# swoonge/SC-A-LOAM

Measured on AMD Instinct MI355X. Metric: scans/sec (feat-extract + scan-to-map ICP + SC loop search), KITTI HDL-64, higher is better.
Workload: dtype f32 points / f64 pose algebra

## Files before the change

sc-a-loam_amd/csrc/mapping.hip:

```cpp
#include "common.hpp"
#include <mutex>
#include <atomic>
#include "device_utils.hpp"
#include "voxel_dev.hpp"
#include "radix_sort.hpp"
#include "lm_host.hpp"
#include "features_dev.hpp"
#include <cmath>
#include <cstdlib>
#include <algorithm>
#include <deque>

namespace scal {

constexpr int CW = 21, CH = 21, CD = 11;
constexpr int GX = 250, GY = 250, GZ = 150;
constexpr int GCELLS = GX * GY * GZ;
constexpr unsigned long long MAP_NOMERGE = 127ull;

struct MapParams {
    int cenW, cenH, cenD;
    int cI, cJ, cK;
    int ox, oy, oz;
    float inv_line, inv_plane;
// ... 663 lines not shown
        C->n_total[cls] = min(n_old + ns, cap);
        if (n_old + ns > cap) C->error = SCAL_E_CAPACITY;
    }
    if (i >= n_old + ns || i >= cap) return;
    float x, y, z;
    int pc;
    if (i < n_old) {
        x = m.x[i], y = m.y[i], z = m.z[i], pc = m.cube[i];
    } else {
        const int j = i - n_old;
        double x7[7];
#pragma unroll
        for (int k = 0; k < 7; ++k) x7[k] = st->x[k];
        float sel[3];
        associate_to_map(x7, stack.x[j], stack.y[j], stack.z[j], sel);
        x = sel[0], y = sel[1], z = sel[2];
        pc = pack_cube(cube_abs(x) , cube_abs(y), cube_abs(z));
        m.x[i] = x, m.y[i] = y, m.z[i] = z, m.w[i] = stack.w[j], m.cube[i] = pc;
    }
    const unsigned long long k = map_key(mp, inv_leaf, x, y, z, pc, C);
    keys[i] = k;
    vals[i] = i;
}
SCAL_KERNEL(256, k_insert_keys)

__device__ __forceinline__ void k_map_heads_body(const SortedPairs& sp, const int* __restrict__ d_n, int* __restrict__ blockcnt) {
    const unsigned long long* keys = sp.keys[sorted_sel(sp)];
    const int n = *d_n;
    const int nb = (n + 255) / 256;
    if (static_cast<int>(blockIdx.x) >= nb) return;
    __shared__ int s[17];
    const int i = blockIdx.x * 256 + threadIdx.x;
    int head = 0;
    if (i < n) {
        const unsigned long long k = keys[i];
        head = (k != ~0ull) && (((k >> 27) == MAP_NOMERGE) || i == 0 || keys[i - 1] != k);
    }
    int total;
    block_exclusive_scan(head, s, &total);
    if (threadIdx.x == 0) blockcnt[blockIdx.x] = total;
}
SCAL_KERNEL(256, k_map_heads)

__device__ __forceinline__ void k_map_reduce_body(const SortedPairs& sp, const int* __restrict__ d_n, const int* __restrict__ blockoff, const MapCloud& in,
                                                    const MapCloud& out) {
    const unsigned long long* keys = sp.keys[sorted_sel(sp)];
    const int* vals = sp.vals[sorted_sel(sp)];
    const int n = *d_n;
    const int nb = (n + 255) / 256;
    if (static_cast<int>(blockIdx.x) >= nb) return;
    __shared__ int s[17];
    const int i = blockIdx.x * 256 + threadIdx.x;
    int head = 0;
    unsigned long long k = 0;
    if (i < n) {
        k = keys[i];
        head = (k != ~0ull) && (((k >> 27) == MAP_NOMERGE) || i == 0 || keys[i - 1] != k);
    }
    int total;
    const int rank = block_exclusive_scan(head, s, &total);
    if (!head) return;
    const int o = blockoff[blockIdx.x] + rank;
    if ((k >> 27) == MAP_NOMERGE) {
        const int g = vals[i];
        out.x[o] = in.x[g], out.y[o] = in.y[g], out.z[o] = in.z[g], out.w[o] = in.w[g], out.cube[o] = in.cube[g];
        return;
    }
    float ax = 0.f, ay = 0.f, az = 0.f, aw = 0.f;
    int u = i;
    while (u < n && keys[u] == k) {
        const int g = vals[u];
        ax += in.x[g], ay += in.y[g], az += in.z[g], aw += in.w[g];
        ++u;
    }
    const float c = static_cast<float>(u - i);
    out.x[o] = ax / c, out.y[o] = ay / c, out.z[o] = az / c, out.w[o] = aw / c;
    out.cube[o] = in.cube[vals[i]];
}
SCAL_KERNEL(256, k_map_reduce)

constexpr int MERGE_MAX = 16384;
constexpr int MERGE_IDX_BITS = 14;
constexpr int MERGE_SAMPLES = 4096;

struct MergeNew {
    float *x, *y, *z, *w;
    int* cube;
    unsigned long long* pkey;
    unsigned long long* sorted;
    unsigned long long* samp;
    int* pre;
    int* lb;
    unsigned char* hm;
    int* blocktot;
};
struct MergeArgs {
    MapCloud in[2], out[2];
    CSoA4 stack[2];
    const int* d_ns[2];
    float inv_leaf[2];
    unsigned long long* okeys[2];
    MergeNew nw[2];
    int cap;
    int2* grid_cell[2];
    const int* grid_rank[2];
    int prebuild;
    int2* next_cell[2];
    int* next_rank[2];
    float4* next_pool[2];
    unsigned long long* next_okeys[2];
    int next_cap[2];
};
constexpr int MERGE_CHUNKS = MERGE_MAX / 512;
constexpr int MERGE_KB0 = 24, MERGE_KB1 = 88;
constexpr int MERGE_KEYS_GRID = 2 * MERGE_CHUNKS;
constexpr int MERGE_NEW_BLOCKS = MERGE_MAX / 256;
constexpr int MERGE_WB0 = 256, MERGE_WB1 = 1536;
constexpr int MERGE_WRITE_GRID = MERGE_WB0 + MERGE_WB1 + 2 * MERGE_NEW_BLOCKS;


__device__ __forceinline__ void k_merge_okeys_body(const MergeArgs& a, const MapState* __restrict__ S, MapCounters* C) {
    if (S->abort) return;
    const MapParams mp = S->mp;
    int b = blockIdx.x;
    const int cls = b < MERGE_KB0 ? 0 : 1;
    const int nblk = cls ? MERGE_KB1 : MERGE_KB0;
    if (cls) b -= MERGE_KB0;
    const MapCloud m = a.in[cls];
    const int n_old = S->n_map[cls];
    for (int i = b * 1024 + threadIdx.x; i < n_old; i += nblk * 1024) {
        const unsigned long long k = map_key(mp, a.inv_leaf[cls], m.x[i], m.y[i], m.z[i], m.cube[i], C);
        a.okeys[cls][i] = k;
        bool bad = k == ~0ull;
        if (i > 0) {
            const unsigned long long kp = map_key(mp, a.inv_leaf[cls], m.x[i - 1], m.y[i - 1], m.z[i - 1], m.cube[i - 1], C);
            bad |= kp > k || (kp == k && !key_nomerge(k));
        }
        if (bad) C->merge_fail = 1;
    }
}
SCAL_KERNEL(1024, k_merge_okeys)

__device__ __forceinline__ void k_merge_keys_body(const MergeArgs& a, const LMState* __restrict__ st, MapState* S, MapCounters* C) {
    if (S->abort) return;
    if (blockIdx.x == 0 && threadIdx.x == 0) S->next_valid[0] = 0, S->next_valid[1] = 0, S->next_unsorted = 0, S->next_over = 0;
    extern __shared__ __align__(16) unsigned long long sk[];
    __shared__ int s_scan[17];
    int b = blockIdx.x;
    const int cls = b / MERGE_CHUNKS, tile = b % MERGE_CHUNKS;
    const int ns = *a.d_ns[cls];
    const int n_new = min(ns, MERGE_MAX);
    const int nc = (n_new + 511) >> 9;
    if (tile == 0 && threadIdx.x == 0 && (ns > MERGE_MAX || S->n_map[cls] + ns > a.cap || !S->window_same)) C->merge_fail = 1;
    if (tile > 0 && tile >= nc) return;
    const MergeNew nw = a.nw[cls];
    int mine = 0;
    for (int i = threadIdx.x; i < nc * 512; i += 1024) {
        const unsigned long long pk = i < n_new ? nw.pkey[i] : ~0ull;
        mine += pk != ~0ull;
        sk[i] = pk;
    }
    int n_eff = 0;
    block_exclusive_scan(mine, s_scan, &n_eff);
    if (tile == 0 && threadIdx.x == 0) C->merge_neff[cls] = n_eff;
    if (nc == 0) return;
    for (int w = wave_id(); w < nc; w += 16) {
        unsigned long long v[8];
        chunk_load(sk, w, v);
        wave_sort512(v);
        chunk_store(sk, w, v);
    }
    __syncthreads();
    const int j = threadIdx.x >> 1, half = threadIdx.x & 1;
    const unsigned long long key = sk[tile * 512 + j];
    int rank = half == 0 ? j : 0;
    for (int c = half; c < nc; c += 2) {
        if (c == tile) continue;
        const unsigned long long* ch = sk + c * 512;
        int lo = 0, hi = 512;
        while (lo < hi) {
            const int mid = (lo + hi) >> 1;
            if (ch[mid] < key) lo = mid + 1;
            else hi = mid;
        }
        rank += lo;
    }
    rank += __shfl_xor(rank, 1, 64);
    if (half == 0 && key != ~0ull) nw.sorted[rank] = key;
}
SCAL_KERNEL(1024, k_merge_keys)

__device__ __forceinline__ void k_merge_lookup_body(const MergeArgs& a, const MapState* __restrict__ S, const MapCounters* __restrict__ C) {
    if (S->abort) return;
    __shared__ unsigned long long s_samp[MERGE_SAMPLES];
    __shared__ int s_scan[17];
    const int cls = blockIdx.x / MERGE_CHUNKS, blk = blockIdx.x % MERGE_CHUNKS;
    const MergeNew nw = a.nw[cls];
    const int n_eff = C->merge_neff[cls];
    if (blk * 512 >= n_eff) {
        if (threadIdx.x == 0) nw.blocktot[blk] = 0;
        return;
    }
    const int n_old = S->n_map[cls];
    const unsigned long long* okeys = a.okeys[cls];
    int stride = 32;
    while ((n_old + stride - 1) / stride > MERGE_SAMPLES) stride <<= 1;
    const int n_samp = (n_old + stride - 1) / stride;
    for (int j = threadIdx.x; j < n_samp; j += 512) s_samp[j] = okeys[static_cast<size_t>(j) * stride];
    const int t = blk * 512 + threadIdx.x;
    unsigned long long key = 0;
    bool head = false, nom = false;
    int lo = 0, hi = 0;
    if (t < n_eff) {
        key = nw.sorted[t] >> MERGE_IDX_BITS;
        nom = key_nomerge(key);
        head = nom || t == 0 || (nw.sorted[t - 1] >> MERGE_IDX_BITS) != key;
        if (head && !nom) hi = n_old;
        if (nom) lo = hi = n_old;
    }
    __syncthreads();
    if (lo < hi) {
        int x = 0, y = n_samp;
        while (x < y) {
            const int mid = (x + y) >> 1;
            if (s_samp[mid] < key) x = mid + 1;
            else y = mid;
        }
        lo = x > 0 ? (x - 1) * stride + 1 : 0;
        hi = min(n_old, x * stride);
        if (lo > hi) lo = hi;
        while (lo < hi) {
            const int mid = (lo + hi) >> 1;
            if (okeys[mid] < key) lo = mid + 1;
            else hi = mid;
        }
    }
    const bool matched = head && !nom && lo < n_old && okeys[lo] == key;
    const int ins = (head && !matched) ? 1 : 0;
    int total = 0;
    const int pre = block_exclusive_scan(ins, s_scan, &total);
    if (t < n_eff) {
        nw.hm[t] = (head ? 1 : 0) | (matched ? 2 : 0);
        nw.lb[t] = lo;
        nw.pre[t] = pre;
        if ((t & 7) == 0) nw.samp[t >> 3] = key;
    }
    if (threadIdx.x == 0) nw.blocktot[blk] = total;
}
SCAL_KERNEL(512, k_merge_lookup)

__device__ __forceinline__ void merge_write_body(const MergeArgs& a, MapState* S, MapCounters* C) {
    if (S->abort) return;
    if (static_cast<int>(blockIdx.x) < MERGE_WB0 + MERGE_WB1) {
        const int cls0 = static_cast<int>(blockIdx.x) < MERGE_WB0 ? 0 : 1;
        const int b0 = cls0 ? blockIdx.x - MERGE_WB0 : blockIdx.x, nblk0 = cls0 ? MERGE_WB1 : MERGE_WB0;
        const MapParams mp0 = S->mp;
        const MapCloud m0 = a.in[cls0];
        const int n0 = S->n_map[cls0];
        for (int i = b0 * 256 + threadIdx.x; i < n0; i += nblk0 * 256)
            if (a.grid_rank[cls0][i] >= 0) a.grid_cell[cls0][grid_cell(mp0, m0.x[i], m0.y[i], m0.z[i])].x = 0;
    }
    if (C->merge_fail) {
        if (blockIdx.x == 0 && threadIdx.x == 0) __hip_atomic_store(&S->abort, static_cast<int>(MAP_ABORT_MERGE), __ATOMIC_RELAXED, __HIP_MEMORY_SCOPE_AGENT);
        return;
    }
    if (static_cast<int>(blockIdx.x) >= MERGE_WRITE_GRID) return;
    __shared__ int s_base[MERGE_CHUNKS + 1];
    __shared__ unsigned long long s_samp[MERGE_MAX / 8];
    int b = blockIdx.x;
    int cls, part, nblk;
    if (b < MERGE_WB0) cls = 0, part = 0, nblk = MERGE_WB0;
    else if ((b -= MERGE_WB0) < MERGE_WB1) cls = 1, part = 0, nblk = MERGE_WB1;
    else if ((b -= MERGE_WB1) < MERGE_NEW_BLOCKS) cls = 0, part = 1, nblk = MERGE_NEW_BLOCKS;
    else b -= MERGE_NEW_BLOCKS, cls = 1, part = 1, nblk = MERGE_NEW_BLOCKS;
    const MapCloud in = a.in[cls], out = a.out[cls];
    const MergeNew nw = a.nw[cls];
    const int n_eff = C->merge_neff[cls];
    const int n_old = S->n_map[cls];
    if (part == 0 && b * 256 >= n_old && b > 0) return;
    const int n_samp = (n_eff + 7) >> 3;
    if (part == 0)
        for (int q = threadIdx.x; q < n_samp; q += 256) s_samp[q] = nw.samp[q];
    if (threadIdx.x < MERGE_CHUNKS) s_base[threadIdx.x + 1] = nw.blocktot[threadIdx.x];
    __shared__ int s_valid;
    if (threadIdx.x == 0) s_valid = 0;
    __syncthreads();
    if (threadIdx.x == 0) {
        int run = 0;
        for (int q = 0; q < MERGE_CHUNKS; ++q) {
            const int v = s_base[q + 1];
            s_base[q] = run;
            run += v;
        }
        s_base[MERGE_CHUNKS] = run;
    }
    __syncthreads();
    const int total = s_base[MERGE_CHUNKS];
    if (n_old + total > a.cap) {
        if (b == 0 && part == 0 && threadIdx.x == 0) __hip_atomic_store(&S->abort, static_cast<int>(MAP_ABORT_MERGE), __ATOMIC_RELAXED, __HIP_MEMORY_SCOPE_AGENT);
        return;
    }
    if (b == 0 && part == 0 && threadIdx.x == 0) __hip_atomic_store(&C->n_map_new[cls], n_old + total, __ATOMIC_RELAXED, __HIP_MEMORY_SCOPE_AGENT);
    auto pre_at = [&](int t) { return t < n_eff ? nw.pre[t] + s_base[t >> 9] : total; };
    const MapParams mp = S->mp;
    bool drifted = false, over = false;
    int n_in = 0;
    auto prebuild = [&](int o, float x, float y, float z, int cube, unsigned long long placed) {
        const unsigned long long k = map_key(mp, a.inv_leaf[cls], x, y, z, cube, C);
        a.next_okeys[cls][o] = k;
        drifted |= k != placed;
        if (cube_valid(mp, cube)) {
            ++n_in;
            const int cap = a.next_cap[cls];
            const int c = grid_cell(mp, x, y, z);
            const int r = atomicAdd(&a.next_cell[cls][c].x, 1);
            a.next_rank[cls][o] = r;
            if (r < cap) {
                a.next_pool[cls][static_cast<size_t>(c) * cap + r] = make_float4(x, y, z, __int_as_float(o));
                if (r == 0) a.next_cell[cls][c].y = c * cap;
            } else {
                over = true;
            }
        } else {
            a.next_rank[cls][o] = -1;
        }
    };
    if (part == 0) {
        for (int i = b * 256 + threadIdx.x; i < n_old; i += nblk * 256) {
            const unsigned long long k = a.okeys[cls][i];
            const float ix = in.x[i], iy = in.y[i], iz = in.z[i], iw = in.w[i];
            const int cube = in.cube[i];
            int lo, hi;
            {
                int x = 0, y = n_samp;
                while (x < y) {
                    const int mid = (x + y) >> 1;
                    if (s_samp[mid] < k) x = mid + 1;
                    else y = mid;
                }
                lo = x > 0 ? (x - 1) * 8 + 1 : 0;
                hi = min(n_eff, x * 8);
                if (lo > hi) lo = hi;
            }
            unsigned long long e[8];
#pragma unroll
            for (int j = 0; j < 8; ++j) e[j] = lo + j < n_eff ? nw.sorted[lo + j] : ~0ull;
            int cn = 0;
#pragma unroll
            for (int j = 0; j < 7; ++j) cn += (lo + j < hi && (e[j] >> MERGE_IDX_BITS) < k) ? 1 : 0;
            const int at = lo + cn;
            const int o = i + pre_at(at);
            float ax = 0.f, ay = 0.f, az = 0.f, aw = 0.f;
            ax += ix, ay += iy, az += iz, aw += iw;
            int cnt = 1;
            if (!key_nomerge(k)) {
                bool run = true;
#pragma unroll
                for (int j = 0; j < 8; ++j)
                    if (j >= cn) {
                        run = run && (e[j] >> MERGE_IDX_BITS) == k;
                        if (run) {
                            const int jn = static_cast<int>(e[j] & (MERGE_MAX - 1));
                            ax += nw.x[jn], ay += nw.y[jn], az += nw.z[jn], aw += nw.w[jn];
                            ++cnt;
                        }
                    }
                if (run) {
                    int u = lo + 8;
                    while (u < n_eff && (nw.sorted[u] >> MERGE_IDX_BITS) == k) {
                        const int jn = static_cast<int>(nw.sorted[u] & (MERGE_MAX - 1));
                        ax += nw.x[jn], ay += nw.y[jn], az += nw.z[jn], aw += nw.w[jn];
                        ++u, ++cnt;
                    }
                }
            }
            const float c = static_cast<float>(cnt);
            const float ox = ax / c, oy = ay / c, oz = az / c;
            out.x[o] = ox, out.y[o] = oy, out.z[o] = oz, out.w[o] = aw / c, out.cube[o] = cube;
            if (a.prebuild) prebuild(o, ox, oy, oz, cube, k);
        }
    } else {
        const int i = b * 256 + threadIdx.x;
        if (i < n_eff && (nw.hm[i] & 3) == 1) {
            const unsigned long long k = nw.sorted[i] >> MERGE_IDX_BITS;
            const int o = nw.lb[i] + pre_at(i);
            float ax = 0.f, ay = 0.f, az = 0.f, aw = 0.f;
// ... 40 lines not shown
    merge_write_body(a, S, C);
    if (!t.fused) return;
    if (static_cast<int>(blockIdx.x) >= MERGE_WRITE_GRID && S->pose_seq == t.seq) {
        const int i = (blockIdx.x - MERGE_WRITE_GRID) * 256 + threadIdx.x;
        if (i < min(*t.d_nfull, t.full_cap)) {
            double x7[7];
#pragma unroll
            for (int k = 0; k < 7; ++k) x7[k] = t.st->x[k];
            float sel[3];
            associate_to_map(x7, t.full.x[i], t.full.y[i], t.full.z[i], sel);
            t.full_out.x[i] = sel[0], t.full_out.y[i] = sel[1], t.full_out.z[i] = sel[2], t.full_out.w[i] = t.full.w[i];
        }
    }
}
SCAL_KERNEL(256, k_merge_write)

__device__ __forceinline__ void k_transform_cloud_body(const CSoA4& in, const int* __restrict__ d_n, int cap, const LMState* __restrict__ st,
                                                         const MapState* __restrict__ S, const SoA4& out) {
    if (S->abort) return;
    const int i = blockIdx.x * blockDim.x + threadIdx.x;
    if (i >= min(*d_n, cap)) return;
    double x7[7];
#pragma unroll
    for (int k = 0; k < 7; ++k) x7[k] = st->x[k];
    float sel[3];
    associate_to_map(x7, in.x[i], in.y[i], in.z[i], sel);
    out.x[i] = sel[0], out.y[i] = sel[1], out.z[i] = sel[2], out.w[i] = in.w[i];
}
SCAL_KERNEL(256, k_transform_cloud)

__device__ __forceinline__ void k_map_gather_body(const float* __restrict__ less_aos, const int* __restrict__ d_n_less, const CSoA4& less_flat,
                                                    const int* __restrict__ d_n_less_flat, const SoA4& corner_in, const SoA4& surf_in, MapCounters* C, int cap,
                                                    int nbc, unsigned* surf_parts) {
    const bool corner = static_cast<int>(blockIdx.x) < nbc;
    const int b = corner ? blockIdx.x : blockIdx.x - nbc;
    const int n = min(corner ? *d_n_less : *d_n_less_flat, cap);
    const int i = b * 256 + threadIdx.x;
    if (blockIdx.x == 0) {
        int* w = reinterpret_cast<int*>(C);
        for (int t = 2 + threadIdx.x; t < static_cast<int>(sizeof(MapCounters) / sizeof(int)); t += 256) w[t] = 0;
    }
    if (i == 0) (corner ? C->n_corner_in : C->n_surf_in) = n;
    if (corner) {
        if (i >= n) return;
        const float4 p = reinterpret_cast<const float4*>(less_aos)[i];
        corner_in.x[i] = p.x, corner_in.y[i] = p.y, corner_in.z[i] = p.z, corner_in.w[i] = p.w;
    } else {
        float x = 0.f, y = 0.f, z = 0.f;
        if (i < n) {
            x = less_flat.x[i], y = less_flat.y[i], z = less_flat.z[i];
            surf_in.x[i] = x, surf_in.y[i] = y, surf_in.z[i] = z, surf_in.w[i] = less_flat.w[i];
        }
        if (surf_parts) vox_bbox_block_store(surf_parts, b, i < n, x, y, z);
    }
}
SCAL_KERNEL(256, k_map_gather)

__device__ __forceinline__ void k_export_valid_body(const MapCloud& m, const MapState* __restrict__ S, int cls, int* __restrict__ counter,
                                                      float* __restrict__ out, int cap) {
    const MapParams mp = S->mp;
    const int n = S->n_map[cls];
    for (int i = blockIdx.x * blockDim.x + threadIdx.x; i < n; i += gridDim.x * blockDim.x)
        if (cube_valid(mp, m.cube[i])) {
            const int p = atomicAdd(counter, 1);
            if (p < cap) reinterpret_cast<float4*>(out)[p] = make_float4(m.x[i], m.y[i], m.z[i], m.w[i]);
        }
}
SCAL_KERNEL(256, k_export_valid)


__device__ __forceinline__ void copy_words(void* dst, const void* src, int bytes) {
    const unsigned* s = static_cast<const unsigned*>(src);
    unsigned* d = static_cast<unsigned*>(dst);
    for (int i = threadIdx.x; i < bytes / 4; i += blockDim.x) d[i] = s[i];
}

struct PoseDoneNew {
    CSoA4 stack[2];
    const int* d_ns[2];
    float inv_leaf[2];
    float *x[2], *y[2], *z[2], *w[2];
    int* cube[2];
    unsigned long long* pkey[2];
};
struct MapPoseDone {
    int active;
    unsigned seq;
    MapState* S;
    const LMState* st;
    MapCounters* C;
    MapResult* host;
    PoseDoneNew nw;
    __device__ __forceinline__ void operator()(const double* x, int first, int stride, bool aborted) const {
        if (!active) return;
        const bool stop = aborted || S->abort;
        if (!stop) {
            const MapParams mp = S->mp;
            double x7[7];
#pragma unroll
            for (int k = 0; k < 7; ++k) x7[k] = x[k];
#pragma unroll
            for (int cls = 0; cls < 2; ++cls) {
                const int n_new = min(*nw.d_ns[cls], MERGE_MAX);
                const CSoA4 stack = nw.stack[cls];
                for (int i = first; i < n_new; i += stride) {
                    float sel[3];
                    associate_to_map(x7, stack.x[i], stack.y[i], stack.z[i], sel);
                    const int pc = pack_cube(cube_abs(sel[0]), cube_abs(sel[1]), cube_abs(sel[2]));
                    const unsigned long long k = map_key(mp, nw.inv_leaf[cls], sel[0], sel[1], sel[2], pc, C);
                    nw.x[cls][i] = sel[0], nw.y[cls][i] = sel[1], nw.z[cls][i] = sel[2], nw.w[cls][i] = stack.w[i], nw.cube[cls][i] = pc;
                    nw.pkey[cls][i] = k == ~0ull ? ~0ull : ((k << MERGE_IDX_BITS) | static_cast<unsigned long long>(i));
                }
            }
        }
        if (blockIdx.x != 0) return;
        if (first == 0 && !stop) {
            const double* q_wodom = S->q_wodom;
            const double n2 = q_wodom[0] * q_wodom[0] + q_wodom[1] * q_wodom[1] + q_wodom[2] * q_wodom[2] + q_wodom[3] * q_wodom[3];
            const double qi[4] = {-q_wodom[0] / n2, -q_wodom[1] / n2, -q_wodom[2] / n2, q_wodom[3] / n2};
            double qn[4];
            q_mul(x, qi, qn);
            double r2[3];
            q_rot(qn, S->t_wodom, r2);
#pragma unroll
            for (int i = 0; i < 4; ++i) S->q_wmap_wodom[i] = qn[i];
#pragma unroll
            for (int i = 0; i < 3; ++i) S->t_wmap_wodom[i] = x[4 + i] - r2[i];
            S->pose_seq = seq;
        }
        __syncthreads();
        copy_words(&host->st, st, sizeof(LMState));
        copy_words(&host->C1, C, sizeof(MapCounters));
        copy_words(&host->S1, S, sizeof(MapState));
        __threadfence_system();
        __syncthreads();
        if (threadIdx.x == 0) __hip_atomic_store(&host->seq_pose, seq, __ATOMIC_RELEASE, __HIP_MEMORY_SCOPE_SYSTEM);
    }
    __device__ __forceinline__ void operator()(int, int, int) const {}
};

__device__ __forceinline__ void k_map_pose_done_body(const MapPoseDone& pd) {
    pd(pd.st->x, blockIdx.x * blockDim.x + threadIdx.x, gridDim.x * blockDim.x, false);
}
SCAL_KERNEL(256, k_map_pose_done)

__device__ __forceinline__ void k_map_end_body(MapState* S, const MapCounters* C, MapResult* host, unsigned seq) {
    if (threadIdx.x == 0 && !S->abort) S->n_map[0] = C->n_map_new[0], S->n_map[1] = C->n_map_new[1];
    __syncthreads();
    copy_words(&host->C2, C, sizeof(MapCounters));
    copy_words(&host->S2, S, sizeof(MapState));
    __threadfence_system();
    __syncthreads();
    if (threadIdx.x == 0) __hip_atomic_store(&host->seq_done, seq, __ATOMIC_RELEASE, __HIP_MEMORY_SCOPE_SYSTEM);
}
SCAL_KERNEL(256, k_map_end)

struct MapStore {
    SoAStore pts[2];
    DevBuf<int> cube[2];
    int n = 0;
    MapCloud cloud(int b) { return MapCloud{pts[b].x.p, pts[b].y.p, pts[b].z.p, pts[b].w.p, cube[b].p}; }
};

struct GridStore {
    DevBuf<int2> cell[2];
    DevBuf<int> rank[2];
    DevBuf<float4> g;
    DevBuf<float4> fixed[2];
    DevBuf<unsigned long long> okeys[2];
    int fixed_cap = 0;
    GridPts pts(int par, bool fixed_pool = false) { return GridPts{fixed_pool ? fixed[par].p : g.p}; }
};

SCAL_DEFINE_STAMP_READER(scal_debug_stamps_map)
}

using namespace scal;
// ... 19 lines not shown
    bool pose_collected = false;
    bool confirmed = false;
    bool failed = false;
    bool prebuilt = false;
    unsigned seq = 0;
    unsigned feat_generation = 0;
    int n_corner_bound = 0, n_surf_bound = 0;
    int insert_path = 0;
};

struct InputSet {
    SoAStore in[2], stack[2];
    DevBuf<MapCounters> C;
    DevBuf<unsigned> surf_parts;
    Event ev_pre;
    Event ev_pre_a;
    int* n_in(int k) const { return k == 0 ? &C.p->n_corner_in : &C.p->n_surf_in; }
    int* n_stack(int k) const { return k == 0 ? &C.p->n_corner_stack : &C.p->n_surf_stack; }
};

template <class T, int N>
struct Fifo {
    T item[N];
    int n = 0;
    void push(const T& v) { item[n++] = v; }
    const T& front() const { return item[0]; }
    void pop() { std::copy(item + 1, item + n, item), --n; }
    void clear() { n = 0; }
};

struct scal_map {
    scal_map_config cfg;
    LaneStream stream;
    LaneStream side;
    static constexpr int NSETS = 8;
    static constexpr int MAX_STEPS = 4;
    static constexpr int MAX_PF = 3;
    static constexpr int NSLOTS = MAX_STEPS + 1;
    struct Prefetch {
        scal_features_t* feat;
        int set;
        unsigned generation;
    };
    std::mutex pf_mu;
    Fifo<Prefetch, MAX_PF> pf_half;
    Fifo<Prefetch, MAX_PF> pf;
    int next_set = 0;
    std::deque<MapStep> steps;
    Event ev_pose[NSLOTS], ev_done[NSLOTS];
    int next_slot = 0;
    PinBuf<MapResult> res;
    bool adapter_active = false;
    MapStep adapter_step;
    BlockAdapter blocks;
    int n_fast = 0, n_general = 0, n_recover_pose = 0, n_recover_insert = 0;
    bool poll_on_enqueue = true;
    int cur = 0;
    bool initialised = false;
    double good_q[4] = {0, 0, 0, 1}, good_t[3] = {0, 0, 0};
    int scan_cap = 0, map_cap = 0;
    double q_wmap_wodom[4] = {0, 0, 0, 1}, t_wmap_wodom[3] = {0, 0, 0};
    bool have_mp = false;
    DevBuf<MapState> d_S;
    DevBuf<float> aos;
    DevBuf<float> export_buf;
    InputSet sets[NSETS];
    SoAStore full_in, full_out;
    float leaf(int k) const { return k == 0 ? cfg.line_res : cfg.plane_res; }
    float inv_leaf(int k) const { return 1.0f / leaf(k); }
    VoxelFilter vf, vf_side, vf_corner;
    MapStore map[2];
    GridStore grid[2];
    HostStage hs_reg;
    bool grid_fixed = false;
    unsigned seq_counter = 0;
    bool grid_prebuilt = false;
    int grid_cap_now[2] = {0, 0};
    RadixSort sorter;
    DevBuf<unsigned long long> keys;
    DevBuf<int> vals, blockcnt;
    bool merge_insert = true;
    int last_insert_path = 0;
    SoAStore mnew[2];
    DevBuf<int> mcube[2], mpre[2], mlb[2], mblocktot[2];
    DevBuf<unsigned long long> msorted[2], mpkey[2], msamp[2];
    DevBuf<unsigned char> mhm[2];
    MergeNew merge_new(int k) {
        return MergeNew{mnew[k].x.p, mnew[k].y.p, mnew[k].z.p, mnew[k].w.p, mcube[k].p, mpkey[k].p, msorted[k].p, msamp[k].p, mpre[k].p, mlb[k].p, mhm[k].p, mblocktot[k].p};
    }
    LMStore lm;
    DevBuf<float> nnrec;
    NNBuf nnbuf() { return NNBuf{nnrec.p, lm.slot_cap}; }
    DevBuf<int> d_nfull;
    PinBuf<MapCounters> h_C;
    PinBuf<MapState> h_S;
    PinBuf<int> h_misc;
    int alloc_set() {
        const int st = next_set;
        next_set = (next_set + 1) % NSETS;
        return st;
    }
};

int scal::map_create(const scal_map_config* cfg, StreamLayout layout, scal_map_t** out) {
    if (!cfg || !out || cfg->max_scan_points <= 0 || cfg->max_map_points <= 0 || !(cfg->line_res > 0) || !(cfg->plane_res > 0)) {
        set_error("scal_map_create: bad argument");
        return SCAL_E_ARG;
    }
    if (cfg->line_res < 0.11f || cfg->plane_res < 0.11f) {
        set_error("mapping resolutions below 0.11 m exceed the 512 voxel/cube key layout");
        return SCAL_E_ARG;
    }
    *out = nullptr;
    SCAL_TRY(select_device(cfg->device));
    auto* c = new scal_map();
    c->cfg = *cfg;
    c->scan_cap = cfg->max_scan_points;
    c->map_cap = cfg->max_map_points;
    int rc = SCAL_OK;
    auto A = [&](int r) { if (rc == SCAL_OK) rc = r; };
    const size_t sc = c->scan_cap, mc = c->map_cap;
    A(c->aos.alloc(sc * 4));
    for (InputSet& I : c->sets) {
        A(I.in[0].alloc(sc)); A(I.in[1].alloc(sc)); A(I.stack[0].alloc(sc)); A(I.stack[1].alloc(sc));
        A(I.C.alloc(1));
        A(I.surf_parts.alloc((size_t)6 * (div_up(c->scan_cap, 256) + 1)));
    }
    A(c->full_in.alloc(sc)); A(c->full_out.alloc(sc));
    A(c->vf.init(c->scan_cap));
    A(c->vf_side.init(c->scan_cap));
    A(c->vf_corner.init(c->scan_cap));
    c->vf.set_tag(".C"), c->vf_side.set_tag(".C"), c->vf_corner.set_tag(".C");
    for (int k = 0; k < 2; ++k) {
        for (int b = 0; b < 2; ++b) {
            A(c->map[k].pts[b].alloc(mc));
            A(c->map[k].cube[b].alloc(mc));
        }
        for (int par = 0; par < 2; ++par) { A(c->grid[k].cell[par].alloc(GCELLS)); A(c->grid[k].rank[par].alloc(mc)); A(c->grid[k].okeys[par].alloc(mc)); }
        A(c->grid[k].g.alloc(mc));
    }
    A(c->sorter.init(c->map_cap));
    A(c->keys.alloc(mc)); A(c->vals.alloc(mc)); A(c->blockcnt.alloc(div_up(c->map_cap, 256) + 1));
    for (int k = 0; k < 2; ++k) {
        A(c->mnew[k].alloc(MERGE_MAX)); A(c->mcube[k].alloc(MERGE_MAX)); A(c->mpre[k].alloc(MERGE_MAX + 1)); A(c->mlb[k].alloc(MERGE_MAX));
        A(c->msorted[k].alloc(MERGE_MAX)); A(c->mhm[k].alloc(MERGE_MAX)); A(c->mblocktot[k].alloc(MERGE_CHUNKS));
        A(c->mpkey[k].alloc(MERGE_MAX)); A(c->msamp[k].alloc(MERGE_MAX / 8));
    }
    A(c->lm.alloc(c->scan_cap));
    A(c->nnrec.alloc(16 * sc));
    A(c->d_S.alloc(1)); A(c->d_nfull.alloc(4));
    A(c->blocks.alloc(c->scan_cap));
    A(c->h_C.alloc(1)); A(c->h_S.alloc(1)); A(c->h_misc.alloc(4)); A(c->res.alloc(scal_map::NSLOTS));
    const char* fixed_env = std::getenv("SCALOAM_MAP_FIXED_GRID");
    if (rc == SCAL_OK && !(fixed_env && fixed_env[0] == '0')) {
        int cap[2];
        for (int k = 0; k < 2; ++k) {
            const int a = voxels_per_cell_axis(c->leaf(k));
            cap[k] = a * a * a;
        }
        if (cap[0] + cap[1] <= 48) {
            c->grid_fixed = true;
            for (int k = 0; k < 2 && c->grid_fixed; ++k) {
                for (int par = 0; par < 2; ++par)
                    if (c->grid[k].fixed[par].alloc(static_cast<size_t>(GCELLS) * cap[k]) != SCAL_OK) c->grid_fixed = false;
                c->grid[k].fixed_cap = c->grid_cap_now[k] = cap[k];
            }
            if (!c->grid_fixed) {
                (void)hipGetLastError();
                for (int k = 0; k < 2; ++k) c->grid[k].fixed[0].release(), c->grid[k].fixed[1].release();
            }
        }
    }
    if (rc == SCAL_OK) std::memset(static_cast<void*>(c->res.p), 0, sizeof(MapResult) * scal_map::NSLOTS);
    if (rc == SCAL_OK) rc = lm_check_residency<AssocFit, MapPoseDone>(c->cfg.device);
    if (rc == SCAL_OK && hipFuncSetAttribute(reinterpret_cast<const void*>(k_merge_keys), hipFuncAttributeMaxDynamicSharedMemorySize,
                                             static_cast<int>(sizeof(unsigned long long) * MERGE_MAX)) != hipSuccess)
        rc = SCAL_E_HIP;
    if (rc == SCAL_OK) rc = c->stream.acquire(c->cfg.device, stage_lane(layout, STAGE_MAP));
    if (rc == SCAL_OK) rc = c->side.acquire(c->cfg.device, stage_lane(layout, STAGE_MAP_PREFETCH));
    for (int k = 0; k < scal_map::NSLOTS && rc == SCAL_OK; ++k) {
        rc = c->ev_pose[k].create(hipEventDisableTiming);
        if (rc == SCAL_OK) rc = c->ev_done[k].create(hipEventDisableTiming);
    }
    if (rc == SCAL_OK) {
        for (int k = 0; k < 4 && rc == SCAL_OK; ++k) rc = c->grid[k & 1].cell[k >> 1].zero(c->stream);
        if (rc == SCAL_OK) rc = c->lm.init(c->stream);
        MapState& H = *c->h_S.p;
        std::memset(&H, 0, sizeof H);
        H.q_wmap_wodom[3] = 1.0;
        H.mp.cenW = 10, H.mp.cenH = 10, H.mp.cenD = 5;
        if (rc == SCAL_OK && op_memcpy_async(c->d_S.p, c->h_S.p, sizeof(MapState), hipMemcpyHostToDevice, c->stream) != hipSuccess) rc = SCAL_E_HIP;
        if (rc == SCAL_OK && op_stream_synchronize(c->stream) != hipSuccess) rc = SCAL_E_HIP;
    }
    if (rc != SCAL_OK) {
        if (rc == SCAL_E_HIP) set_error("scal_map_create: HIP resource creation failed");
        delete c;
        return rc;
    }
    *out = c;
    return SCAL_OK;
}

extern "C" int scal_map_create(const scal_map_config* cfg, scal_map_t** out) { return map_create(cfg, default_stream_layout(), out); }

extern "C" void scal_map_destroy(scal_map_t* c) {
    if (!c) return;
    (void)hipSetDevice(c->cfg.device);
    if (c->stream) (void)op_stream_synchronize(c->stream);
    if (c->side) (void)op_stream_synchronize(c->side);
    delete c;
}

namespace {

void copy_pose(double* q, double* t, const double* q_from, const double* t_from) {
    std::copy(q_from, q_from + 4, q);
    std::copy(t_from, t_from + 3, t);
}

int enqueue_stack_filter(scal_map* c, int k, VoxelFilter& vf, hipStream_t s, int n_bound, int st, bool surf_box_done = false) {
    InputSet& I = c->sets[st];
    VoxTail t;
    t.err_out = &I.C.p->error;
    const int bits = c->leaf(k) >= 0.35f ? 30 : 40;
    const bool box = k == 1 && surf_box_done && n_bound > 8192;
    return vf.run(s, I.in[k].cv(), I.n_in(k), n_bound, c->leaf(k), bits, I.stack[k].v(), I.n_stack(k), &t, box ? I.surf_parts.p : nullptr,
                  box ? std::max(1, div_up(n_bound, 256)) : 0);
}

GridArgs grid_args(scal_map* c, int par, bool fixed_pool = false) {
    GridArgs ga;
    for (int k = 0; k < 2; ++k) {
        GridStore& G = c->grid[k];
        ga.m[k] = c->map[k].cloud(par);
        ga.cell[k] = G.cell[par].p, ga.rank[k] = G.rank[par].p, ga.g[k] = G.pts(par, fixed_pool);
        ga.okeys[k] = G.okeys[par].p;
        ga.inv_leaf[k] = c->inv_leaf(k);
    }
    return ga;
}

int insert_full_sort(scal_map* c, const MapStep& e, const int* n_map) {
    hipStream_t s = c->stream;
    const InputSet& I = c->sets[e.set];
    MapCounters* C = I.C.p;
    LMState* st = c->lm.d_st.p;
    for (int k = 0; k < 2; ++k) {
        MapStore& M = c->map[k];
        const int n_tot_max = std::min(c->map_cap, n_map[k] + c->scan_cap);
        const int nb = std::max(1, div_up(n_tot_max, 256));
        MapCloud in = M.cloud(e.par), outc = M.cloud(e.par ^ 1);
        SCAL_LAUNCH("k_insert_keys", k_insert_keys, dim3(nb), dim3(256), 0, s, in, c->d_S.p, I.stack[k].cv(), I.n_stack(k), st, c->inv_leaf(k),
                           c->map_cap, c->keys.p, c->vals.p, C, k);
        SortedPairs sp;
        SCAL_TRY(c->sorter.sort(s, c->keys.p, c->vals.p, &C->n_total[k], n_tot_max, 36, nullptr, &sp));
        SCAL_LAUNCH("k_map_heads", k_map_heads, dim3(nb), dim3(256), 0, s, sp, &C->n_total[k], c->blockcnt.p);
        launch_scan_inplace(s, c->blockcnt.p, &C->n_total[k], 256, 1, &C->n_map_new[k]);
        SCAL_LAUNCH("k_map_reduce", k_map_reduce, dim3(nb), dim3(256), 0, s, sp, &C->n_total[k], c->blockcnt.p, in, outc);
    }
    SCAL_HIP(hipGetLastError());
    return SCAL_OK;
}

struct FullCloud {
    CSoA4 pts;
    const int* d_n;
};
FullCloud full_cloud(scal_map* c, const MapStep& e) {
    if (!(e.have_full && e.feat)) return FullCloud{c->full_in.cv(), c->d_nfull.p};
    FeatDeviceView v = features_view(e.feat);
    return FullCloud{CSoA4{v.x, v.y, v.z, v.i}, &v.P->n_kept};
}

int launch_insert_merge(scal_map* c, const MapStep& e, bool fused = false) {
    hipStream_t s = c->stream;
    const InputSet& I = c->sets[e.set];
    MapCounters* C = I.C.p;
    MergeArgs a;
    for (int k = 0; k < 2; ++k) {
        MapStore& M = c->map[k];
        a.in[k] = M.cloud(e.par), a.out[k] = M.cloud(e.par ^ 1);
        a.stack[k] = I.stack[k].cv();
        a.d_ns[k] = I.n_stack(k);
        a.inv_leaf[k] = c->inv_leaf(k);
        GridStore& G = c->grid[k];
        a.okeys[k] = G.okeys[e.par].p;
        a.nw[k] = c->merge_new(k);
        a.grid_cell[k] = G.cell[e.par].p, a.grid_rank[k] = G.rank[e.par].p;
        a.next_cell[k] = G.cell[e.par ^ 1].p, a.next_rank[k] = G.rank[e.par ^ 1].p, a.next_pool[k] = G.fixed[e.par ^ 1].p;
        a.next_okeys[k] = G.okeys[e.par ^ 1].p, a.next_cap[k] = c->grid_cap_now[k];
    }
    a.prebuild = fused && c->grid_fixed ? 1 : 0;
    a.cap = c->map_cap;
    const int lds = sizeof(unsigned long long) * MERGE_MAX;
    if (!(fused && c->grid_fixed)) SCAL_LAUNCH("k_merge_okeys", k_merge_okeys, dim3(MERGE_KB0 + MERGE_KB1), dim3(1024), 0, s, a, c->d_S.p, C);
    SCAL_LAUNCH("k_merge_keys", k_merge_keys, dim3(MERGE_KEYS_GRID), dim3(1024), lds, s, a, c->lm.d_st.p, c->d_S.p, C);
    SCAL_LAUNCH("k_merge_lookup", k_merge_lookup, dim3(2 * MERGE_CHUNKS), dim3(512), 0, s, a, c->d_S.p, C);
    MergeTail t{};
    int grid = MERGE_WRITE_GRID;
    if (fused) {
        t.fused = 1, t.seq = e.seq, t.st = c->lm.d_st.p, t.full_out = c->full_out.v(), t.full_cap = c->scan_cap;
        const FullCloud f = full_cloud(c, e);
        t.full = f.pts, t.d_nfull = f.d_n;
        if (e.have_full) grid += std::max(1, div_up(c->scan_cap, 256));
        else t.full_cap = 0;
    }
    SCAL_LAUNCH("k_merge_write", k_merge_write, dim3(grid), dim3(256), 0, s, a, c->d_S.p, C, t);
    SCAL_HIP(hipGetLastError());
    return SCAL_OK;
}

void launch_grid_clear(scal_map* c, int par) {
    SCAL_LAUNCH("k_grid_clear", k_grid_clear, dim3(GRID_BLOCKS), dim3(256), 0, c->stream, grid_args(c, par), c->d_S.p);
}
int clear_abort(scal_map* c) {
    hipStream_t s = c->stream;
    SCAL_HIP(op_memset_async(&c->d_S.p->abort, 0, sizeof(int), s));
    return SCAL_OK;
}
void launch_map_end(scal_map* c, const MapStep& e) {
    SCAL_LAUNCH("k_map_end", k_map_end, dim3(1), dim3(256), 0, c->stream, c->d_S.p, c->sets[e.set].C.p, c->res.p + e.slot, e.seq);
}
bool stopped_before_pose(const MapResult& R) { return R.S1.abort || R.st.termination == 5; }
bool stopped_in_insertion(const MapResult& R) { return R.S2.abort != 0; }

int launch_tail(scal_map* c, const MapStep& e, bool registered = false) {
    hipStream_t s = c->stream;
    if (e.have_full && !registered) {
        const int nb = std::max(1, div_up(c->scan_cap, 256));
        const FullCloud f = full_cloud(c, e);
        SCAL_LAUNCH("k_transform_cloud", k_transform_cloud, dim3(nb), dim3(256), 0, s, f.pts, f.d_n, c->scan_cap, c->lm.d_st.p, c->d_S.p, c->full_out.v());
    }
    launch_map_end(c, e);
    SCAL_HIP(hipGetLastError());
    SCAL_HIP(op_event_record(c->ev_done[e.slot], s));
    if (e.feat && !registered) SCAL_TRY(features_note_reader(e.feat, s));
    return SCAL_OK;
}

MapPoseDone make_pose_done(scal_map* c, const MapStep& e) {
    const InputSet& I = c->sets[e.set];
    MapPoseDone pd;
    pd.active = 1, pd.seq = e.seq;
    pd.S = c->d_S.p, pd.st = c->lm.d_st.p, pd.C = I.C.p, pd.host = c->res.p + e.slot;
    for (int k = 0; k < 2; ++k) {
        pd.nw.stack[k] = I.stack[k].cv();
        pd.nw.d_ns[k] = I.n_stack(k);
        pd.nw.inv_leaf[k] = c->inv_leaf(k);
        pd.nw.x[k] = c->mnew[k].x.p, pd.nw.y[k] = c->mnew[k].y.p, pd.nw.z[k] = c->mnew[k].z.p, pd.nw.w[k] = c->mnew[k].w.p;
        pd.nw.cube[k] = c->mcube[k].p, pd.nw.pkey[k] = c->mpkey[k].p;
    }
    return pd;
}

int launch_pose_part(scal_map* c, const MapStep& e, bool prepare_only = false) {
    hipStream_t s = c->stream;
    const int st_ = e.set;
    InputSet& I = c->sets[st_];
    MapCounters* C = I.C.p;
    LMState* st = c->lm.d_st.p;
    MapState* S = c->d_S.p;
    if (e.feat) {
        if (e.prefetched) {
            SCAL_HIP(op_stream_wait_event(s, I.ev_pre, 0));
        } else {
            FeatDeviceView v = features_view(e.feat);
            SCAL_TRY(features_wait_done(e.feat, s));
            const int nbc = std::max(1, div_up(e.n_corner_bound, 256));
            SCAL_LAUNCH("k_map_gather", k_map_gather, dim3(nbc + std::max(1, div_up(e.n_surf_bound, 256))), dim3(256), 0, s, v.less_xyzi, &v.P->n_less_sharp,
                               CSoA4{v.lfx, v.lfy, v.lfz, v.lfi}, &v.P->n_less_flat, I.in[0].v(), I.in[1].v(), C, c->scan_cap, nbc,
                               static_cast<unsigned*>(nullptr));
        }
    }
    if (!e.prefetched) {
        SCAL_TRY(enqueue_stack_filter(c, 0, c->vf, s, e.n_corner_bound, st_));
        SCAL_TRY(enqueue_stack_filter(c, 1, c->vf, s, e.n_surf_bound, st_));
    }
    MapBeginArgs mb;
    mb.active = 0, mb.in = e.pose, mb.allow_window_change = e.fast ? 0 : 1, mb.inv_line = c->inv_leaf(0), mb.inv_plane = c->inv_leaf(1);
    mb.slot_cap = c->lm.slot_cap, mb.prebuilt = e.prebuilt ? 1 : 0, mb.S = S;
    const bool begin_in_knn = e.fast && e.prebuilt && c->grid_fixed && !prepare_only;
    if (!begin_in_knn) SCAL_LAUNCH("k_map_begin", k_map_begin, dim3(1), dim3(64), 0, s, mb, st, C);
    const bool fixed_pool = e.fast && c->grid_fixed && !prepare_only;
    const GridArgs ga = grid_args(c, e.par, fixed_pool);
    if (fixed_pool) {
        if (!e.prebuilt) SCAL_LAUNCH("k_grid_build", k_grid_build, dim3(GRID_BLOCKS), dim3(256), 0, s, ga, c->grid_cap_now[0], c->grid_cap_now[1], S, C);
    } else {
        SCAL_LAUNCH("k_grid_count", k_grid_count, dim3(GRID_BLOCKS), dim3(256), 0, s, ga, S, C);
        SCAL_LAUNCH("k_grid_alloc", k_grid_alloc, dim3(GRID_BLOCKS), dim3(256), 0, s, ga, S, C);
        SCAL_LAUNCH("k_grid_fill", k_grid_fill, dim3(GRID_BLOCKS), dim3(256), 0, s, ga, S);
    }
    if (prepare_only) {
        SCAL_HIP(hipGetLastError());
        return SCAL_OK;
    }
    FactorSoA F = c->lm.factors();
    const int assoc_blocks = std::max(1, std::min(3072, div_up(c->lm.slot_cap, 8)));
    MapPoseDone pd = make_pose_done(c, e);
    const AssocFit fit{I.stack[0].cv(), I.stack[1].cv(), c->nnbuf(), C, F};
    for (int outer = 0; outer < 2; ++outer) {
        {
            mb.active = (begin_in_knn && outer == 0) ? 1 : 0;
            SCAL_LAUNCH(mb.active ? "k_assoc_knn.0" : "k_assoc_knn", k_assoc_knn, dim3(assoc_blocks), dim3(256), 0, s, I.stack[0].cv(), I.stack[1].cv(), S,
                             c->grid[0].cell[e.par].p, c->grid[0].pts(e.par, fixed_pool), c->grid[1].cell[e.par].p, c->grid[1].pts(e.par, fixed_pool), st, C, c->nnbuf(), mb);
        }
        pd.active = outer == 1;
        launch_lm_solve(s, F, &C->n_slots, st, &C->solve_on, c->lm.partials.p, c->lm.lm_sync.p, outer, &S->abort, fit, pd, "k_lm_solve_map");
    }
    SCAL_HIP(hipGetLastError());
    if (!e.fast) SCAL_HIP(op_event_record(c->ev_pose[e.slot], s));
    return SCAL_OK;
}

static bool step_flag_set(const volatile unsigned* w, unsigned seq) {
    if (*w != seq) return false;
    std::atomic_thread_fence(std::memory_order_acquire);
    return true;
}
static int step_flag_wait(scal_map* c, const volatile unsigned* w, unsigned seq) {
    if (g_recorder) SCAL_HIP(op_flush_for_wait(__FILE__, __LINE__));
    for (unsigned spins = 0;; ++spins) {
        if (step_flag_set(w, seq)) return SCAL_OK;
        if ((spins & 0xfff) == 0xfff && hipStreamQuery(c->stream) == hipSuccess) {
            if (step_flag_set(w, seq)) return SCAL_OK;
            set_error("scal_map: the stream is idle and the step never reported (a kernel launch failed?)");
            return SCAL_E_HIP;
        }
        __builtin_ia32_pause();
    }
}
static int wait_pose(scal_map* c, const MapStep& e) {
    if (e.fast) return step_flag_wait(c, &c->res.p[e.slot].seq_pose, e.seq);
    SCAL_HIP(op_event_synchronize(c->ev_pose[e.slot]));
// ... 748 lines not shown
```

Baseline: 4449.

## Fold merge lookup into merge_keys kernel and replace block scan with insert bitmask

The separate k_merge_lookup kernel is removed. Its work now runs inside k_merge_keys: each thread takes its predecessor key from the chunk binary searches, does the old-map lookup there, and writes sorted/hm/lb/samp at its final rank. The per-block prefix scan and blocktot array are replaced by a global bitmask of insert flags, set with atomicOr and cleared in the pose-done functor. k_merge_write then builds offsets with popcount plus a wave-level scan. This saves one kernel launch and a round trip through global memory, at the cost of atomics and a mask clear that must run before every merge.

```diff
diff --git a/sc-a-loam_amd/csrc/mapping.hip b/sc-a-loam_amd/csrc/mapping.hip
--- a/sc-a-loam_amd/csrc/mapping.hip
+++ b/sc-a-loam_amd/csrc/mapping.hip
@@ -769,6 +769,7 @@
 constexpr int MERGE_MAX = 16384;
 constexpr int MERGE_IDX_BITS = 14;
 constexpr int MERGE_SAMPLES = 4096;
+constexpr int MERGE_MASK_WORDS = MERGE_MAX / 64;
 
 struct MergeNew {
     float *x, *y, *z, *w;
@@ -776,10 +777,9 @@
     unsigned long long* pkey;
     unsigned long long* sorted;
     unsigned long long* samp;
-    int* pre;
     int* lb;
     unsigned char* hm;
-    int* blocktot;
+    unsigned long long* mask;
 };
 struct MergeArgs {
     MapCloud in[2], out[2];
@@ -859,49 +859,40 @@
     }
     __syncthreads();
     const int j = threadIdx.x >> 1, half = threadIdx.x & 1;
-    const unsigned long long key = sk[tile * 512 + j];
+    const unsigned long long pk = sk[tile * 512 + j];
     int rank = half == 0 ? j : 0;
+    unsigned long long prev = (half == 0 && j > 0) ? sk[tile * 512 + j - 1] : 0ull;
     for (int c = half; c < nc; c += 2) {
         if (c == tile) continue;
         const unsigned long long* ch = sk + c * 512;
         int lo = 0, hi = 512;
         while (lo < hi) {
             const int mid = (lo + hi) >> 1;
-            if (ch[mid] < key) lo = mid + 1;
+            if (ch[mid] < pk) lo = mid + 1;
             else hi = mid;
         }
         rank += lo;
+        if (lo > 0) prev = max(prev, ch[lo - 1]);
     }
     rank += __shfl_xor(rank, 1, 64);
-    if (half == 0 && key != ~0ull) nw.sorted[rank] = key;
-}
-SCAL_KERNEL(1024, k_merge_keys)
-
-__device__ __forceinline__ void k_merge_lookup_body(const MergeArgs& a, const MapState* __restrict__ S, const MapCounters* __restrict__ C) {
-    if (S->abort) return;
-    __shared__ unsigned long long s_samp[MERGE_SAMPLES];
-    __shared__ int s_scan[17];
-    const int cls = blockIdx.x / MERGE_CHUNKS, blk = blockIdx.x % MERGE_CHUNKS;
-    const MergeNew nw = a.nw[cls];
-    const int n_eff = C->merge_neff[cls];
-    if (blk * 512 >= n_eff) {
-        if (threadIdx.x == 0) nw.blocktot[blk] = 0;
-        return;
-    }
+    {
+        const unsigned lo32 = __shfl_xor(static_cast<unsigned>(prev), 1, 64), hi32 = __shfl_xor(static_cast<unsigned>(prev >> 32), 1, 64);
+        prev = max(prev, (static_cast<unsigned long long>(hi32) << 32) | lo32);
+    }
+    const bool live = half == 0 && pk != ~0ull;
+    __syncthreads();
     const int n_old = S->n_map[cls];
     const unsigned long long* okeys = a.okeys[cls];
     int stride = 32;
     while ((n_old + stride - 1) / stride > MERGE_SAMPLES) stride <<= 1;
     const int n_samp = (n_old + stride - 1) / stride;
-    for (int j = threadIdx.x; j < n_samp; j += 512) s_samp[j] = okeys[static_cast<size_t>(j) * stride];
-    const int t = blk * 512 + threadIdx.x;
-    unsigned long long key = 0;
+    for (int q = threadIdx.x; q < n_samp; q += 1024) sk[q] = okeys[static_cast<size_t>(q) * stride];
+    const unsigned long long key = pk >> MERGE_IDX_BITS;
     bool head = false, nom = false;
     int lo = 0, hi = 0;
-    if (t < n_eff) {
-        key = nw.sorted[t] >> MERGE_IDX_BITS;
+    if (live) {
         nom = key_nomerge(key);
-        head = nom || t == 0 || (nw.sorted[t - 1] >> MERGE_IDX_BITS) != key;
+        head = nom || rank == 0 || (prev >> MERGE_IDX_BITS) != key;
         if (head && !nom) hi = n_old;
         if (nom) lo = hi = n_old;
     }
@@ -910,7 +901,7 @@
         int x = 0, y = n_samp;
         while (x < y) {
             const int mid = (x + y) >> 1;
-            if (s_samp[mid] < key) x = mid + 1;
+            if (sk[mid] < key) x = mid + 1;
             else y = mid;
         }
         lo = x > 0 ? (x - 1) * stride + 1 : 0;
@@ -922,19 +913,16 @@
             else hi = mid;
         }
     }
+    if (!live) return;
     const bool matched = head && !nom && lo < n_old && okeys[lo] == key;
-    const int ins = (head && !matched) ? 1 : 0;
-    int total = 0;
-    const int pre = block_exclusive_scan(ins, s_scan, &total);
-    if (t < n_eff) {
-        nw.hm[t] = (head ? 1 : 0) | (matched ? 2 : 0);
-        nw.lb[t] = lo;
-        nw.pre[t] = pre;
-        if ((t & 7) == 0) nw.samp[t >> 3] = key;
-    }
-    if (threadIdx.x == 0) nw.blocktot[blk] = total;
-}
-SCAL_KERNEL(512, k_merge_lookup)
+    nw.sorted[rank] = pk;
+    nw.hm[rank] = (head ? 1 : 0) | (matched ? 2 : 0);
+    nw.lb[rank] = lo;
+    if ((rank & 7) == 0) nw.samp[rank >> 3] = key;
+    if (head && !matched) atomicOr(&nw.mask[rank >> 6], 1ull << (rank & 63));
+}
+SCAL_KERNEL(1024, k_merge_keys)
+
 
 __device__ __forceinline__ void merge_write_body(const MergeArgs& a, MapState* S, MapCounters* C) {
     if (S->abort) return;
@@ -952,7 +940,8 @@
         return;
     }
     if (static_cast<int>(blockIdx.x) >= MERGE_WRITE_GRID) return;
-    __shared__ int s_base[MERGE_CHUNKS + 1];
+    __shared__ int s_pre[MERGE_MASK_WORDS + 1];
+    __shared__ unsigned long long s_mask[MERGE_MASK_WORDS];
     __shared__ unsigned long long s_samp[MERGE_MAX / 8];
     int b = blockIdx.x;
     int cls, part, nblk;
@@ -968,27 +957,35 @@
     const int n_samp = (n_eff + 7) >> 3;
     if (part == 0)
         for (int q = threadIdx.x; q < n_samp; q += 256) s_samp[q] = nw.samp[q];
-    if (threadIdx.x < MERGE_CHUNKS) s_base[threadIdx.x + 1] = nw.blocktot[threadIdx.x];
+    static_assert(MERGE_MASK_WORDS == 256, "one mask word per thread, four per lane of the scanning wave");
+    s_mask[threadIdx.x] = nw.mask[threadIdx.x];
     __shared__ int s_valid;
     if (threadIdx.x == 0) s_valid = 0;
     __syncthreads();
-    if (threadIdx.x == 0) {
-        int run = 0;
-        for (int q = 0; q < MERGE_CHUNKS; ++q) {
-            const int v = s_base[q + 1];
-            s_base[q] = run;
-            run += v;
-        }
-        s_base[MERGE_CHUNKS] = run;
+    if (threadIdx.x < 64) {
+        const int l = threadIdx.x;
+        int c[4], sum = 0;
+#pragma unroll
+        for (int q = 0; q < 4; ++q) c[q] = __popcll(s_mask[4 * l + q]), sum += c[q];
+        int inc = sum;
+#pragma unroll
+        for (int o = 1; o < 64; o <<= 1) {
+            const int v = __shfl_up(inc, o, 64);
+            if (l >= o) inc += v;
+        }
+        int run = inc - sum;
+#pragma unroll
+        for (int q = 0; q < 4; ++q) s_pre[4 * l + q] = run, run += c[q];
+        if (l == 63) s_pre[MERGE_MASK_WORDS] = run;
     }
     __syncthreads();
-    const int total = s_base[MERGE_CHUNKS];
+    const int total = s_pre[MERGE_MASK_WORDS];
     if (n_old + total > a.cap) {
         if (b == 0 && part == 0 && threadIdx.x == 0) __hip_atomic_store(&S->abort, static_cast<int>(MAP_ABORT_MERGE), __ATOMIC_RELAXED, __HIP_MEMORY_SCOPE_AGENT);
         return;
     }
     if (b == 0 && part == 0 && threadIdx.x == 0) __hip_atomic_store(&C->n_map_new[cls], n_old + total, __ATOMIC_RELAXED, __HIP_MEMORY_SCOPE_AGENT);
-    auto pre_at = [&](int t) { return t < n_eff ? nw.pre[t] + s_base[t >> 9] : total; };
+    auto pre_at = [&](int t) { return t < n_eff ? s_pre[t >> 6] + __popcll(s_mask[t >> 6] & ((1ull << (t & 63)) - 1ull)) : total; };
     const MapParams mp = S->mp;
     bool drifted = false, over = false;
     int n_in = 0;
@@ -1195,6 +1192,7 @@
     float *x[2], *y[2], *z[2], *w[2];
     int* cube[2];
     unsigned long long* pkey[2];
+    unsigned long long* mask[2];
 };
 struct MapPoseDone {
     int active;
@@ -1206,6 +1204,7 @@
     PoseDoneNew nw;
     __device__ __forceinline__ void operator()(const double* x, int first, int stride, bool aborted) const {
         if (!active) return;
+        for (int i = first; i < 2 * MERGE_MASK_WORDS; i += stride) nw.mask[i / MERGE_MASK_WORDS][i % MERGE_MASK_WORDS] = 0ull;
         const bool stop = aborted || S->abort;
         if (!stop) {
             const MapParams mp = S->mp;
@@ -1391,11 +1390,11 @@
     bool merge_insert = true;
     int last_insert_path = 0;
     SoAStore mnew[2];
-    DevBuf<int> mcube[2], mpre[2], mlb[2], mblocktot[2];
-    DevBuf<unsigned long long> msorted[2], mpkey[2], msamp[2];
+    DevBuf<int> mcube[2], mlb[2];
+    DevBuf<unsigned long long> msorted[2], mpkey[2], msamp[2], mmask[2];
     DevBuf<unsigned char> mhm[2];
     MergeNew merge_new(int k) {
-        return MergeNew{mnew[k].x.p, mnew[k].y.p, mnew[k].z.p, mnew[k].w.p, mcube[k].p, mpkey[k].p, msorted[k].p, msamp[k].p, mpre[k].p, mlb[k].p, mhm[k].p, mblocktot[k].p};
+        return MergeNew{mnew[k].x.p, mnew[k].y.p, mnew[k].z.p, mnew[k].w.p, mcube[k].p, mpkey[k].p, msorted[k].p, msamp[k].p, mlb[k].p, mhm[k].p, mmask[k].p};
     }
     LMStore lm;
     DevBuf<float> nnrec;
@@ -1451,8 +1450,8 @@
     A(c->sorter.init(c->map_cap));
     A(c->keys.alloc(mc)); A(c->vals.alloc(mc)); A(c->blockcnt.alloc(div_up(c->map_cap, 256) + 1));
     for (int k = 0; k < 2; ++k) {
-        A(c->mnew[k].alloc(MERGE_MAX)); A(c->mcube[k].alloc(MERGE_MAX)); A(c->mpre[k].alloc(MERGE_MAX + 1)); A(c->mlb[k].alloc(MERGE_MAX));
-        A(c->msorted[k].alloc(MERGE_MAX)); A(c->mhm[k].alloc(MERGE_MAX)); A(c->mblocktot[k].alloc(MERGE_CHUNKS));
+        A(c->mnew[k].alloc(MERGE_MAX)); A(c->mcube[k].alloc(MERGE_MAX)); A(c->mlb[k].alloc(MERGE_MAX));
+        A(c->msorted[k].alloc(MERGE_MAX)); A(c->mhm[k].alloc(MERGE_MAX)); A(c->mmask[k].alloc(MERGE_MASK_WORDS));
         A(c->mpkey[k].alloc(MERGE_MAX)); A(c->msamp[k].alloc(MERGE_MAX / 8));
     }
     A(c->lm.alloc(c->scan_cap));
@@ -1604,7 +1603,6 @@
     const int lds = sizeof(unsigned long long) * MERGE_MAX;
     if (!(fused && c->grid_fixed)) SCAL_LAUNCH("k_merge_okeys", k_merge_okeys, dim3(MERGE_KB0 + MERGE_KB1), dim3(1024), 0, s, a, c->d_S.p, C);
     SCAL_LAUNCH("k_merge_keys", k_merge_keys, dim3(MERGE_KEYS_GRID), dim3(1024), lds, s, a, c->lm.d_st.p, c->d_S.p, C);
-    SCAL_LAUNCH("k_merge_lookup", k_merge_lookup, dim3(2 * MERGE_CHUNKS), dim3(512), 0, s, a, c->d_S.p, C);
     MergeTail t{};
     int grid = MERGE_WRITE_GRID;
     if (fused) {
@@ -1657,7 +1655,7 @@
         pd.nw.d_ns[k] = I.n_stack(k);
         pd.nw.inv_leaf[k] = c->inv_leaf(k);
         pd.nw.x[k] = c->mnew[k].x.p, pd.nw.y[k] = c->mnew[k].y.p, pd.nw.z[k] = c->mnew[k].z.p, pd.nw.w[k] = c->mnew[k].w.p;
-        pd.nw.cube[k] = c->mcube[k].p, pd.nw.pkey[k] = c->mpkey[k].p;
+        pd.nw.cube[k] = c->mcube[k].p, pd.nw.pkey[k] = c->mpkey[k].p, pd.nw.mask[k] = c->mmask[k].p;
     }
     return pd;
 }
```

Result: no change. 4494 (median of 2 runs) (+1.0%).
